# microsoft/MoGe

Hardware: AMD Instinct MI355X
Metric: images/sec (MoGeModel.infer, moge-2-vitl 518x518 fp16) (higher is better)
Workload: dtype f16; 1 GPU; moge-2-vitl infer(): batch 32/GPU x 3x518x518 torch.rand, num_tokens 3600, fp16 weights, synthetic checkpoint (seed 0), inputs resident in HBM, outputs left on device; global_batch=32, parallelism=dp1 (independent shards, one-time RCCL weight broadcast)

## Files before the change

include/moge_hip.h:

```cpp
#ifndef MOGE_HIP_H
#define MOGE_HIP_H

#include <stddef.h>
#include <stdint.h>

#ifdef __cplusplus
extern "C" {
#endif

#define MOGE_ABI_VERSION 5
#define MOGE_MAX_TAPS 8
#define MOGE_LEVELS 5

typedef enum moge_status {
    MOGE_OK = 0,
    MOGE_ERR_INVALID = -1,
    MOGE_ERR_HIP = -2,
    MOGE_ERR_NOT_LOADED = -3,
    MOGE_ERR_MISSING_KEY = -4,
    MOGE_ERR_NONFINITE = -5
} moge_status;

typedef enum moge_precision {
    MOGE_FP32 = 0,
// ... 124 lines not shown
int moge_cast_f16(const float* src, void* dst_f16, int64_t n, void* stream);

int moge_sync(moge_handle* h, void* stream);

int moge_profile_enable(moge_handle* h, int on);
int moge_profile_read(moge_handle* h, moge_profile* out, int reset);

int moge_debug_tap(moge_handle* h, const char* name, float* dst, int64_t dst_capacity, int64_t* numel, void* stream);

void moge_tune_set(const char* key, int value);

int moge_test_gemm(int precision, const float* A, const float* W, const float* bias, float* C, int M, int N, int K,
                   int act, void* stream);
enum { MOGE_TG_STORE = 0, MOGE_TG_RESID = 1, MOGE_TG_QKV = 2, MOGE_TG_CONVT = 3, MOGE_TG_PATCH = 4 };
typedef struct moge_test_gemm_args {
    int32_t precision, kind, act;
    int32_t M, N, K;
    const float* A; const float* W; const float* bias;
    float* out;
    const float* ln_mr; const float* ln_c;
    const float* wu; const float* wv; float u0, u1, v0, v1;
    int32_t pixW, pixH, Cout;
    float* xres; const float* gamma; float* x16_out; float* ln_part_out;
    float* q_out; float* k_out; float* v_out; int32_t nh, Ntok; float qscale;
    const float* pos; const float* cls; int32_t Np;
    int32_t v_transposed;
    int32_t uv_in;
} moge_test_gemm_args;
int moge_test_gemm_ex(const moge_test_gemm_args* args, void* stream);
int moge_test_layernorm(int precision, const float* x, const float* w, const float* b, float* y, int rows, int D, void* stream);
int moge_test_attention(int precision, const float* q, const float* k, const float* v, float* o, int B, int nh, int N, void* stream);
int moge_test_conv3x3(int precision, const float* x, const float* w, const float* bias, float* y, int B, int H, int W,
                      int Cin, int Cout, int relu_in, void* stream);
typedef struct moge_test_conv_args {
    int32_t precision, B, H, W, Cin, Cout;
    int32_t relu_in, act, up2;
    const float* x; const float* w; const float* bias;
    const float* add;
    const float* side; const float* side_w;
    const float* wu; const float* wv; float u0, u1, v0, v1;
    const float* w2; const float* bias2;
    float* y;
    const float* dot_w; int32_t dot_rows;
} moge_test_conv_args;
int moge_test_conv_ex(const moge_test_conv_args* args, void* stream);
typedef struct moge_test_ct3_args {
    int32_t precision, B, H, W, Cin, Cout, no_border;
    const float* x; const float* wt; const float* bt; const float* w3; const float* b3;
    const float* side; const float* side_w;
    const float* wu; const float* wv; float u0, u1, v0, v1;
    float* y;
} moge_test_ct3_args;
int moge_test_ct3(const moge_test_ct3_args* args, void* stream);
int moge_test_convt2x2(int precision, const float* x, const float* w, const float* bias, float* y, int B, int H, int W,
                       int Cin, int Cout, void* stream);
int moge_test_preprocess(const float* image, float* out, int B, int H, int W, int rows, int cols, void* stream);
int moge_test_preprocess_ex(int in_fp16, int out_fp16, const float* image, float* out, int32_t* zero_i32, int B, int H, int W, int rows, int cols, int ldk,
                            int nchw_out, int round16, int aa, int zero_n, void* stream);
int moge_test_resize_bicubic_aa(const float* image, float* out, int B, int H, int W, int OH, int OW, void* stream);
int moge_test_resize_bicubic_aa_ex(int in_fp16, const float* image, float* out, int B, int H, int W, int OH, int OW, int round16, void* stream);
int moge_test_groupnorm_relu(int precision, const float* x, const float* gamma, const float* beta, float* y, int B, int H, int W, int C, int groups, void* stream);
int moge_test_norm_act(int precision, const float* x, const float* gamma, const float* beta, float* y, int B, int H, int W, int C, int groups, int act, int in_place, void* stream);
int moge_test_posembed(const float* pos, float* out, int D, int rows, int cols, void* stream);
int moge_test_posembed_ex(const float* pos, float* out, int D, int rows, int cols, int size_mode, void* stream);
int moge_test_recover(const float* points, const uint8_t* mask, const float* focal_in, int B, int H, int W,
                      float* focal, float* shift, int32_t* status, void* stream);
typedef struct moge_test_head_args {
    int32_t precision, kind, remap, ksize;
    int32_t B, Hd, Wd, C, ld, choff, H, W;
    int32_t n4_below;
    const float* x; const float* w; const float* bias;
    const float* n4; const float* w2;
    float* out;
} moge_test_head_args;
int moge_test_head_final(const moge_test_head_args* args, void* stream);
int moge_test_head_final_dot(int kind, int remap, const float* y, const float* z, int zld, int zoff, const float* bias, float* out, int B, int Hd, int Wd,
                             int H, int W, void* stream);
int moge_test_mlp_layer(const float* in, const float* W, const float* bias, float* out, int B, int K, int N, int act, void* stream);
int moge_test_layernorm_ex(int precision, int stream16, const float* x, const float* w, const float* b, float* y, float* cls_out, int rows, int D, int ldo,
                           int coloff, int tap_mode, int Ntok, void* stream);
int moge_test_ln_raw(const float* x, float* x16_out, float* mr, int rows, int D, void* stream);
int moge_test_ln_finalize(const float* part, float* mr, int rows, int NP, int D, void* stream);
int moge_test_fold_ln(const float* W, const float* g, const float* beta, const float* b, float* Wf_out, float* c, float* bf, int N, int K, void* stream);
int moge_test_resize_bilinear_uv(int precision, const float* x, float* out, int B, int hs, int ws, int C, int OH, int OW, int Cp, float u0, float u1,
                                 float v0, float v1, void* stream);
int moge_test_u8_ingest(int precision, const uint8_t* in, float* out, int B, int H, int W, void* stream);

int moge_align_l1(const float* x, const float* y, const float* w, int rows, int n, float eps, float* a, float* loss, int32_t* index, void* stream);
int moge_align_l1_anchored(const float* src, const float* tgt, const float* weight, int n, int d, int comp_mask, const int32_t* row_batch,
                           const int32_t* row_anchor, int rows, float eps, float* scale, float* loss, int32_t* index, void* stream);
int moge_align_trunc_workspace(int n, int rows, int64_t* bytes);
int moge_align_trunc(const float* x, const float* y, const float* w, int rows, int n, float trunc, float eps, void* workspace, float* a, float* loss,
                     int32_t* index, void* stream);
int moge_align_trunc_anchored(const float* src, const float* tgt, const float* weight, int n, int d, int comp_mask, const int32_t* row_batch,
                              const int32_t* row_anchor, int rows, float trunc, float eps, void* workspace, float* scale, float* loss, int32_t* index,
                              void* stream);
int moge_align_select(const float* loss, const int32_t* row_batch, int rows, int batch, float* min_loss, int32_t* min_row, void* stream);
int moge_align_lstsq(const float* x, const float* y, const float* w, int rows, int n, float* a, float* b, void* stream);

#define MOGE_METRICS_PARTIALS 256
#define MOGE_METRICS_MAX_SEGMENTS 512
int moge_metrics_lr_sample(const uint8_t* mask, int H, int W, int out_h, int out_w, uint8_t* lr_mask, int32_t* lr_index, void* stream);
int moge_metrics_error(const float* pred, const float* gt, const uint8_t* mask, int n, int dim, const float* params, int K, double* partials,
                       double* out, void* stream);
int moge_metrics_masked_max(const float* x, const uint8_t* mask, int n, float* partials, float* out, void* stream);
int moge_metrics_boundary(const float* pred, const float* gt, const uint8_t* mask, int H, int W, int64_t* counts, void* stream);
// ... 46 lines not shown
```

moge_amd/_lib.py:

```python
from __future__ import annotations

import ctypes as C
import os

import torch

HERE = os.path.dirname(os.path.abspath(__file__))
LIB_PATH = os.path.join(HERE, "lib", "libmoge_hip.so")
EXPERIMENTS_LIB_PATH = os.path.join(HERE, "lib", "experiments", "libmoge_hip.so")

MOGE_MAX_TAPS = 8
MOGE_LEVELS = 5
FP32, FP16, FP16_HALF = 0, 1, 2
HEAD_POINTS, HEAD_NORMAL, HEAD_MASK, HEAD_SCALE = 1, 2, 4, 8
FORCE_PROJECTION, APPLY_MASK = 1, 2
REMAP = {"linear": 0, "sinh": 1, "exp": 2, "sinh_exp": 3}
RESAMPLER = {"conv_transpose": 0, "bilinear": 1, "nearest": 2, "pixel_shuffle": 3}
RES_NORM = {"none": 0, "layer_norm": 1, "group_norm": 2, "instance_norm": 3}
ACTIVATION = {"relu": 0, "leaky_relu": 1, "silu": 2, "elu": 3}
ERR_NONFINITE = -5
KC_NAMES = ["gemm", "attn", "conv", "norm", "pre", "post", "recover", "gemm_pp"]
ABI_VERSION = 5
MESH_MAX_MAPS, MESH_BLOCK_PX, MESH_SCAN_SPAN, MESH_NO_FACES = 8, 1024, 256, -1
MESH_F32, MESH_U8, MESH_UV = 0, 1, 2
# ... 62 lines not shown
                ("B", C.c_int32), ("Hd", C.c_int32), ("Wd", C.c_int32), ("C", C.c_int32), ("ld", C.c_int32), ("choff", C.c_int32), ("H", C.c_int32), ("W", C.c_int32),
                ("n4_below", C.c_int32), ("x", C.c_void_p), ("w", C.c_void_p), ("bias", C.c_void_p), ("n4", C.c_void_p), ("w2", C.c_void_p), ("out", C.c_void_p)]


class MeshMap(C.Structure):
    _fields_ = [("data", C.c_void_p), ("out", C.c_void_p), ("channels", C.c_int32), ("dtype", C.c_int32), ("has_scale", C.c_int32),
                ("has_offset", C.c_int32), ("scale", C.c_float * 4), ("offset", C.c_float * 4)]


class MogeError(RuntimeError):
    pass


def _load(path: str = LIB_PATH, mode: int = C.RTLD_GLOBAL) -> C.CDLL:
    if not os.path.exists(path):
        raise ImportError(f"{path} is missing: build it with `python -m moge_amd.build` (hipcc, gfx950). "
                          "moge_amd has no CPU / PyTorch fallback.")
    lib = C.CDLL(path, mode=mode)
    vp, i32, i64, f32p = C.c_void_p, C.c_int, C.c_int64, C.c_void_p
    sig = {
        "moge_abi_version": (C.c_int, []),
        "moge_last_error": (C.c_char_p, []),
        "moge_create": (C.c_int, [C.POINTER(MogeConfig), i32, C.POINTER(vp)]),
        "moge_create_v1": (C.c_int, [C.POINTER(MogeV1Config), i32, C.POINTER(vp)]),
        "moge_v1_forward": (C.c_int, [vp, vp, i32, i32, i32, i32, i32, i32, C.POINTER(Outputs), vp]),
        "moge_v1_infer": (C.c_int, [vp, vp, i32, i32, i32, i32, i32, i32, vp, i32, C.POINTER(Outputs), vp]),
        "moge_destroy": (None, [vp]),
        "moge_load_weights": (C.c_int, [vp, C.POINTER(TensorDesc), i32, vp]),
        "moge_alloc_master": (C.c_int, [vp]),
        "moge_master_blob": (C.c_int, [vp, C.POINTER(vp), C.POINTER(C.c_size_t)]),
        "moge_master_ready": (C.c_int, [vp]),
        "moge_broadcast_weights": (C.c_int, [vp, vp, i32, vp]),
        "moge_set_precision": (C.c_int, [vp, i32, vp]),
        "moge_set_onnx_compatible_mode": (C.c_int, [vp, i32]),
        "moge_workspace_bytes": (C.c_int, [vp, i32, i32, i32, i32, i32, C.POINTER(C.c_size_t)]),
        "moge_forward": (C.c_int, [vp, vp, i32, i32, i32, i32, i32, i32, C.POINTER(Outputs), vp]),
        "moge_infer": (C.c_int, [vp, vp, i32, i32, i32, i32, i32, i32, vp, i32, C.POINTER(Outputs), vp]),
        "moge_postprocess": (C.c_int, [vp, vp, vp, vp, vp, i32, i32, i32, vp, i32, C.POINTER(Outputs), vp]),
        "moge_depth_edge_mask": (C.c_int, [vp, vp, vp, i32, i32, i32, C.c_float, vp, vp]),
        "moge_cast_f16": (C.c_int, [vp, vp, C.c_int64, vp]),
        "moge_sync": (C.c_int, [vp, vp]),
        "moge_profile_enable": (C.c_int, [vp, i32]),
        "moge_profile_read": (C.c_int, [vp, C.POINTER(Profile), i32]),
        "moge_debug_tap": (C.c_int, [vp, C.c_char_p, vp, i64, C.POINTER(i64), vp]),
        "moge_tune_set": (None, [C.c_char_p, i32]),
        "moge_test_gemm": (C.c_int, [i32, f32p, f32p, f32p, f32p, i32, i32, i32, i32, vp]),
        "moge_test_gemm_ex": (C.c_int, [C.POINTER(TestGemmArgs), vp]),
        "moge_test_layernorm": (C.c_int, [i32, f32p, f32p, f32p, f32p, i32, i32, vp]),
        "moge_test_attention": (C.c_int, [i32, f32p, f32p, f32p, f32p, i32, i32, i32, vp]),
        "moge_test_conv3x3": (C.c_int, [i32, f32p, f32p, f32p, f32p, i32, i32, i32, i32, i32, i32, vp]),
        "moge_test_conv_ex": (C.c_int, [C.POINTER(TestConvArgs), vp]),
        "moge_test_convt2x2": (C.c_int, [i32, f32p, f32p, f32p, f32p, i32, i32, i32, i32, i32, vp]),
        "moge_test_ct3": (C.c_int, [C.POINTER(TestCt3Args), vp]),
        "moge_test_preprocess": (C.c_int, [f32p, f32p, i32, i32, i32, i32, i32, vp]),
        "moge_test_preprocess_ex": (C.c_int, [i32, i32, f32p, f32p, vp, i32, i32, i32, i32, i32, i32, i32, i32, i32, i32, vp]),
        "moge_test_resize_bicubic_aa": (C.c_int, [f32p, f32p, i32, i32, i32, i32, i32, vp]),
        "moge_test_resize_bicubic_aa_ex": (C.c_int, [i32, f32p, f32p, i32, i32, i32, i32, i32, i32, vp]),
        "moge_test_groupnorm_relu": (C.c_int, [i32, f32p, f32p, f32p, f32p, i32, i32, i32, i32, i32, vp]),
        "moge_test_norm_act": (C.c_int, [i32, f32p, f32p, f32p, f32p, i32, i32, i32, i32, i32, i32, i32, vp]),
        "moge_test_posembed": (C.c_int, [f32p, f32p, i32, i32, i32, vp]),
        "moge_test_posembed_ex": (C.c_int, [f32p, f32p, i32, i32, i32, i32, vp]),
        "moge_test_recover": (C.c_int, [f32p, vp, f32p, i32, i32, i32, f32p, f32p, vp, vp]),
        "moge_test_head_final": (C.c_int, [C.POINTER(TestHeadArgs), vp]),
        "moge_test_head_final_dot": (C.c_int, [i32, i32, f32p, f32p, i32, i32, f32p, f32p, i32, i32, i32, i32, i32, vp]),
        "moge_test_mlp_layer": (C.c_int, [f32p, f32p, f32p, f32p, i32, i32, i32, i32, vp]),
        "moge_test_layernorm_ex": (C.c_int, [i32, i32, f32p, f32p, f32p, f32p, f32p, i32, i32, i32, i32, i32, i32, vp]),
        "moge_test_ln_raw": (C.c_int, [f32p, f32p, f32p, i32, i32, vp]),
        "moge_test_ln_finalize": (C.c_int, [f32p, f32p, i32, i32, i32, vp]),
        "moge_test_fold_ln": (C.c_int, [f32p, f32p, f32p, f32p, f32p, f32p, f32p, i32, i32, vp]),
        "moge_test_resize_bilinear_uv": (C.c_int, [i32, f32p, f32p, i32, i32, i32, i32, i32, i32, i32, C.c_float, C.c_float, C.c_float, C.c_float, vp]),
        "moge_test_u8_ingest": (C.c_int, [i32, vp, f32p, i32, i32, i32, vp]),
        "moge_align_l1": (C.c_int, [f32p, f32p, f32p, i32, i32, C.c_float, f32p, f32p, vp, vp]),
        "moge_align_l1_anchored": (C.c_int, [f32p, f32p, f32p, i32, i32, i32, vp, vp, i32, C.c_float, f32p, f32p, vp, vp]),
        "moge_align_trunc_workspace": (C.c_int, [i32, i32, C.POINTER(i64)]),
        "moge_align_trunc": (C.c_int, [f32p, f32p, f32p, i32, i32, C.c_float, C.c_float, vp, f32p, f32p, vp, vp]),
        "moge_align_trunc_anchored": (C.c_int, [f32p, f32p, f32p, i32, i32, i32, vp, vp, i32, C.c_float, C.c_float, vp, f32p, f32p, vp, vp]),
        "moge_align_select": (C.c_int, [f32p, vp, i32, i32, f32p, vp, vp]),
        "moge_align_lstsq": (C.c_int, [f32p, f32p, f32p, i32, i32, f32p, f32p, vp]),
        "moge_metrics_lr_sample": (C.c_int, [vp, i32, i32, i32, i32, vp, vp, vp]),
        "moge_metrics_error": (C.c_int, [vp, vp, vp, i32, i32, vp, i32, vp, vp, vp]),
        "moge_metrics_masked_max": (C.c_int, [vp, vp, i32, vp, vp, vp]),
        "moge_metrics_boundary": (C.c_int, [vp, vp, vp, i32, i32, vp, vp]),
        "moge_metrics_segment_stats": (C.c_int, [vp, vp, vp, i32, i32, vp, vp, i32, i32, vp, i32, vp, vp, vp, vp]),
        "moge_metrics_segment_pack": (C.c_int, [vp, i32, vp, vp, i32, i32, vp, i32, vp, i32, i32, vp, vp, vp, vp, vp, vp, vp]),
        "moge_metrics_segment_error": (C.c_int, [vp, vp, vp, vp, i32, vp, i32, vp, vp, i32, vp, vp, vp, vp, vp, vp]),
        "moge_eval_lanczos_workspace": (C.c_int, [i32, i32, i32, i32, vp, vp]),
        "moge_eval_lanczos": (C.c_int, [vp, i32, i32, i32, i32, vp, vp, vp, vp]),
        "moge_eval_masked_nearest": (C.c_int, [vp, vp, i32, i32, i32, i32, C.c_float, C.c_float, C.c_float, C.c_float, vp, vp, vp, vp]),
        "moge_eval_resize_nearest": (C.c_int, [vp, i32, i32, i32, i32, i32, vp, vp]),
        "moge_eval_remap": (C.c_int, [vp, vp, vp, vp, i32, i32, i32, i32, i32, f32p, vp, vp, vp, vp, vp, vp, vp]),
        "moge_eval_quantile_cut": (C.c_int, [vp, vp, i32, C.c_float, C.c_float, C.c_float, i32, vp, vp, vp]),
        "moge_eval_unproject": (C.c_int, [vp, vp, i32, i32, f32p, vp, vp, vp]),
        "moge_refine_depth_workspace": (C.c_int, [i32, i32, i32, C.POINTER(i64)]),
        "moge_refine_depth": (C.c_int, [f32p, f32p, f32p, vp, i32, i32, i32, i32, i32, C.c_float, C.c_float, vp, f32p, vp]),
        "moge_image_mesh_workspace": (C.c_int, [i32, i32, i32, C.POINTER(i64)]),
        "moge_image_mesh_count": (C.c_int, [vp, i32, i32, i32, i32, vp, vp, vp, vp]),
        "moge_image_mesh_fill": (C.c_int, [i32, i32, i32, vp, C.POINTER(MeshMap), i32, i32, vp, vp, vp]),
    }
    for name, (res, args) in sig.items():
        fn = getattr(lib, name)
        fn.restype = res
        fn.argtypes = args
    if lib.moge_abi_version() != ABI_VERSION:
        raise ImportError("libmoge_hip.so ABI version mismatch")
    return lib


lib = _load()
_experiments_lib = None


def experiments_lib() -> C.CDLL:
    global _experiments_lib
    if _experiments_lib is None:
        _experiments_lib = _load(EXPERIMENTS_LIB_PATH, C.RTLD_LOCAL)
    return _experiments_lib
EXPORTS = ["moge_abi_version", "moge_last_error", "moge_create", "moge_create_v1", "moge_v1_forward", "moge_v1_infer", "moge_destroy", "moge_load_weights", "moge_alloc_master",
           "moge_master_blob", "moge_master_ready", "moge_broadcast_weights", "moge_set_precision", "moge_set_onnx_compatible_mode", "moge_workspace_bytes", "moge_forward", "moge_infer",
           "moge_postprocess", "moge_depth_edge_mask", "moge_cast_f16", "moge_sync", "moge_profile_enable", "moge_profile_read", "moge_debug_tap", "moge_tune_set", "moge_test_gemm",
           "moge_test_gemm_ex", "moge_test_layernorm", "moge_test_attention", "moge_test_conv3x3", "moge_test_conv_ex", "moge_test_convt2x2", "moge_test_ct3", "moge_test_preprocess",
           "moge_test_resize_bicubic_aa", "moge_test_groupnorm_relu", "moge_test_norm_act", "moge_test_posembed", "moge_test_recover",
           "moge_test_head_final", "moge_test_head_final_dot", "moge_test_mlp_layer", "moge_test_layernorm_ex", "moge_test_ln_raw", "moge_test_ln_finalize",
           "moge_test_fold_ln", "moge_test_resize_bilinear_uv", "moge_test_u8_ingest",
           "moge_test_preprocess_ex", "moge_test_posembed_ex", "moge_test_resize_bicubic_aa_ex",
           "moge_align_l1", "moge_align_l1_anchored", "moge_align_trunc_workspace", "moge_align_trunc", "moge_align_trunc_anchored",
           "moge_align_select", "moge_align_lstsq",
           "moge_metrics_lr_sample", "moge_metrics_error", "moge_metrics_masked_max", "moge_metrics_boundary", "moge_metrics_segment_stats",
           "moge_metrics_segment_pack", "moge_metrics_segment_error",
           "moge_eval_lanczos_workspace", "moge_eval_lanczos", "moge_eval_masked_nearest", "moge_eval_resize_nearest", "moge_eval_remap",
           "moge_eval_quantile_cut", "moge_eval_unproject",
           "moge_refine_depth_workspace", "moge_refine_depth",
           "moge_image_mesh_workspace", "moge_image_mesh_count", "moge_image_mesh_fill"]


def check(code: int) -> None:
    if code == 0:
        return
    msg = (lib.moge_last_error() or b"").decode(errors="replace")
    if code == ERR_NONFINITE:
        raise ValueError(msg or "Residuals are not finite in the initial point.")
    raise MogeError(f"libmoge_hip error {code}: {msg}")


def tune(key: str, value: int) -> None:
    lib.moge_tune_set(key.encode(), int(value))


def stream_ptr(device=None) -> int:
    return int(torch.cuda.current_stream(device).cuda_stream)


class DevView:

    def __init__(self, ptr: int, nbytes: int):
        self.__cuda_array_interface__ = {"shape": (nbytes,), "typestr": "|u1", "data": (ptr, False), "version": 2, "strides": None}
```

moge_amd/csrc/conv_pp.hip:

```cpp
#include "common.h"

#define CP_GPTR(p) ((const __attribute__((address_space(1))) void*)(p))
__device__ __forceinline__ unsigned cp_opaque(unsigned v) { asm volatile("" : "+v"(v)); return v; }
#define CP_LPTR(p) ((__attribute__((address_space(3))) void*)(p))

namespace {

template <int TW> struct Halo {
    static constexpr int W = TW + 2;
    static constexpr int PX = 18 * W;
    static constexpr int PIECES = (PX + 7) / 8;
    static constexpr int BYTES = PIECES * 1024;
    static constexpr int HPW = (PIECES + 7) / 8;
};

__device__ __forceinline__ u32x4 relu8(u32x4 v) {
#pragma unroll
    for (int i = 0; i < 4; i++) {
        unsigned t = v[i];
        asm("v_pk_max_f16 %0, %0, 0" : "+v"(t));
        v[i] = t;
    }
    return v;
}

template <int N> __device__ __forceinline__ void wait_vm_lgkm() { asm volatile("s_waitcnt vmcnt(%0) lgkmcnt(0)" ::"n"(N) : "memory"); }

template <int BN, int TW, int NH, int EPI>
__global__ __launch_bounds__(512, (BN == 64 && TW == 16 && NH == 1) ? 4 : 2) void conv_pp_kernel(const GemmArgs g) {
    constexpr bool CONVT = (EPI & 2) != 0, HAS_UV = (EPI & 1) != 0, RELU_IN = (EPI & 4) != 0;
    constexpr bool M16 = (EPI & 8) != 0;
    static_assert(!M16 || TW == 16, "16x16x32 path: 16-pixel-wide tiles");
    constexpr bool SIDE_REG = (EPI & 16) != 0;
    constexpr bool DOT = (EPI & 32) != 0;
    static_assert(!DOT || (CONVT && M16 && BN == 128), "fused output conv: the 64 -> 4 x 32 pixel-shuffle resampler");
    constexpr bool CT3 = (EPI & 64) != 0;
    static_assert(!CT3 || (CONVT && M16 && !DOT && !RELU_IN && !SIDE_REG && NH == 2), "fused ConvTranspose2d + 3x3: pixel-shuffle store, 16x16x32 form, two halo buffers");
    constexpr int NTAP = CT3 ? 4 : 9;
    static_assert(!SIDE_REG || (M16 && BN == 64 && NH == 1), "register side input: single-image 64-channel form");
    constexpr int WN = BN / 64, WM = 8 / WN, TM = TW * 16 / 32 / WM, TN = 2;
    constexpr int HALO_W = Halo<TW>::W, HALO_PX = Halo<TW>::PX, HALO_PIECES = Halo<TW>::PIECES, HALO_BYTES = Halo<TW>::BYTES, HPW = Halo<TW>::HPW;
    constexpr int LOG_TW = TW == 16 ? 4 : 5;
    constexpr bool PERSIST = !(BN == 64 && NH == 1);
    constexpr int NWP = BN / 64;
    constexpr int WSLOT = BN * 128;
    constexpr int LDS_W = NH * HALO_BYTES;
    constexpr int WROWS = TM * 32;
    extern __shared__ __attribute__((aligned(16))) char smem[];

    const int tid = threadIdx.x, lane = tid & 63;
    const int wave = __builtin_amdgcn_readfirstlane(tid >> 6);
    const int grp = wave >> 2;
    const int hi = lane >> 5, l31 = lane & 31;
    const int wm = wave / WN, wn = wave % WN;

    const int H = g.H, W = g.W, C = g.C;
    const int tx_n = (W + TW - 1) / TW, ty_n = (H + 15) >> 4;
    const int nbn = g.N / BN;
    int li, cnt, start, wgs_x;
    {
        const int nwg = gridDim.x;
        const int ntiles = PERSIST ? (g.M / (H * W)) * ty_n * tx_n * nbn : nwg;
        const int nx = nwg < 8 ? nwg : 8, xcd = blockIdx.x % nx;
        const int q = ntiles / nx, r = ntiles % nx;
        cnt = q + (xcd < r ? 1 : 0);
        start = xcd * q + min(xcd, r);
        wgs_x = (nwg - xcd + nx - 1) / nx;
        li = blockIdx.x / nx;
    }
    if (li >= cnt) return;
    int b, y0, x0, n0;
    const int nchunks = NH == 1 ? 1 : (C >> 6);
    const int C2 = CT3 ? g.Cout : C;
    const int nside = SIDE_REG ? 1 : ((NH > 1 && g.a2) ? (C2 >> 6) : 0);
    const int nkt1 = nchunks * NTAP;
    const int nkt = nkt1 + nside;

    const int prow = lane >> 3, pch = lane & 7;
    const char* in_b;
    const char* in2_b;
    const char* w_b;
    const char* w2_b;
    unsigned hoff[HPW];
    unsigned hoff2[CT3 ? HPW : 1];
    int sb, sy0, sx0, sn0;
    auto setup = [&](int idx) {
        int prow_t = prow, pch_t = pch;
        if constexpr (PERSIST) asm volatile("" : "+v"(prow_t), "+v"(pch_t));
        const int wgt = start + idx;
        const int bn_ = wgt % nbn;
        int t = wgt / nbn;
        const int tx = t % tx_n; t /= tx_n;
        const int ty = t % ty_n;
        sb = t / ty_n; sy0 = ty * 16; sx0 = tx * TW; sn0 = bn_ * BN;
        in_b = reinterpret_cast<const char*>(g.a) + (size_t)sb * H * W * C * 2;
        in2_b = reinterpret_cast<const char*>(g.a2) + (size_t)sb * H * W * C2 * (CT3 ? 8 : 2);
        w_b = reinterpret_cast<const char*>(g.w) + (size_t)sn0 * g.ldw * 2;
        w2_b = reinterpret_cast<const char*>(g.w2) + (CT3 ? (size_t)0 : (size_t)sn0 * C * 2);
        const int spy = CT3 ? (sn0 / BN) >> 1 : 0, spx = CT3 ? (sn0 / BN) & 1 : 0;
#pragma unroll
        for (int i = 0; i < HPW; i++) {
            int piece = wave + 8 * i;
            piece = piece < HALO_PIECES ? piece : HALO_PIECES - 1;
            int hp = piece * 8 + prow_t;
            const int sw = ((EPI & 8) ? (hp % HALO_W) : ((hp % HALO_W) >> 1)) & 7;
            hp = hp < HALO_PX ? hp : HALO_PX - 1;
            const int hy = hp / HALO_W, hx = hp - hy * HALO_W;
            int yy = sy0 - 1 + hy, xx = sx0 - 1 + hx;
            yy = yy < 0 ? 0 : (yy > H - 1 ? H - 1 : yy);
            xx = xx < 0 ? 0 : (xx > W - 1 ? W - 1 : xx);
            hoff[i] = (unsigned)(((yy * W + xx) * C) * 2 + ((pch_t ^ sw) << 4));
            if constexpr (CT3) hoff2[i] = (unsigned)((((2 * yy + spy) * (2 * W) + 2 * xx + spx) * C2) * 2 + ((pch_t ^ sw) << 4));
        }
    };
    int wrow[NWP];
    unsigned wsw[NWP];
#pragma unroll
    for (int i = 0; i < NWP; i++) {
        wrow[i] = (wave + 8 * i) * 8 + prow;
        wsw[i] = (unsigned)((pch ^ ((wrow[i] >> 1) & 7)) << 4);
    }
    auto issue_halo = [&](int c) {
        char* dst = smem + (c & (NH - 1)) * HALO_BYTES;
        const char* src = uniform_ptr(c < nchunks ? in_b + (size_t)c * 128 : in2_b + (size_t)(c - nchunks) * 128);
        const bool side2 = CT3 && c >= nchunks;
#pragma unroll
        for (int i = 0; i < HPW; i++) {
            int piece = wave + 8 * i;
            piece = piece < HALO_PIECES ? piece : HALO_PIECES - 1;
            unsigned off = hoff[i];
            if constexpr (CT3) off = side2 ? hoff2[i] : off;
            __builtin_amdgcn_global_load_lds(CP_GPTR(src + cp_opaque(off)), CP_LPTR(dst + piece * 1024), 16, 0, 0);
        }
    };
    auto issue_w = [&](int kt) {
        char* dst = smem + LDS_W + (kt & 3) * WSLOT;
        const bool side = kt >= nkt1;
        const int c = CT3 ? kt >> 2 : kt / 9, tap = CT3 ? kt & 3 : kt - c * 9;
        const char* src = uniform_ptr(side ? w2_b + (size_t)(kt - nkt1) * 128 : w_b + ((size_t)tap * C + c * 64) * 2);
        const int rowb = side ? C2 * 2 : g.ldw * 2;
#pragma unroll
        for (int i = 0; i < NWP; i++) {
            const unsigned off = (unsigned)(wrow[i] * rowb) + wsw[i];
            __builtin_amdgcn_global_load_lds(CP_GPTR(src + cp_opaque(off)), CP_LPTR(dst + (wave + 8 * i) * 1024), 16, 0, 0);
        }
    };

    int hp0[TM], hx0[TM];
#pragma unroll
    for (int i = 0; i < TM; i++) {
        const int mp = wm * WROWS + i * 32 + l31;
        hx0[i] = (mp & (TW - 1)) + 1;
        hp0[i] = ((mp >> LOG_TW) + 1) * HALO_W + hx0[i];
    }
    const int sxw = (l31 >> 1) & 7;
    const int w_off = (wn * 64 + l31) * 128 + ((hi ^ sxw) << 4);
    const int l15 = lane & 15, g4 = lane >> 4;
    const int w_off16 = (wn * 64 + l15) * 128 + ((g4 ^ ((l15 >> 1) & 7)) << 4);

    f32x16 acc[TM][TN];
    f32x4 acc16[2 * TM][4];
    const int ntot = nchunks + nside;
    int kt = 0, halo_age = 2;
    int l15t = l15;
    int abase[3][2];
    int tpy = 0;
    auto set_abase = [&]() {
        const bool ph2 = CT3 && BN == 2 * g.Cout;
        const int tpx = CT3 ? (ph2 ? wn : (n0 / BN) & 1) : 0;
        if constexpr (CT3) tpy = ph2 ? (n0 / BN) & 1 : (n0 / BN) >> 1;
#pragma unroll
        for (int d = 0; d < 3; d++) {
            const int hx = l15t + (CT3 ? (d == 2 ? 1 : tpx + d) : d);
            const int a = wm * (2 * TM * HALO_W * 128) + hx * 128 + ((g4 ^ (hx & 7)) << 4);
            abase[d][0] = a; abase[d][1] = a ^ 64;
        }
    };
    u32x4 sidef[SIDE_REG ? 2 * TM : 1][2];
    auto kstep = [&](const char* halo, int dy, int dx, bool first_of_image, int image, bool relu, bool from_regs = false) {
        const char* wsl = smem + LDS_W + (kt & 3) * WSLOT;
        u32x4 af[TM][4], wf[TN][4];
        if constexpr (M16) {
            if (from_regs) {
                if constexpr (SIDE_REG) {
#pragma unroll
                    for (int i = 0; i < 2 * TM; i++)
#pragma unroll
                        for (int ks = 0; ks < 2; ks++) af[i >> 1][(i & 1) * 2 + ks] = sidef[i][ks];
                }
            } else {
#pragma unroll
            for (int i = 0; i < 2 * TM; i++) {
#pragma unroll
                for (int ks = 0; ks < 2; ks++)
                    af[i >> 1][(i & 1) * 2 + ks] = *reinterpret_cast<const u32x4*>(halo + abase[dx + 1][ks] + (i + 1 + dy) * (HALO_W * 128));
            }
            }
#pragma unroll
            for (int j = 0; j < 4; j++)
#pragma unroll
                for (int ks = 0; ks < 2; ks++) wf[j >> 1][(j & 1) * 2 + ks] = *reinterpret_cast<const u32x4*>(wsl + (w_off16 ^ (ks * 64)) + j * 2048);
        } else {
#pragma unroll
        for (int i = 0; i < TM; i++) {
            const int hp = hp0[i] + dy * HALO_W + dx;
            const int a0 = hp * 128 + ((hi ^ (((hx0[i] + dx) >> 1) & 7)) << 4);
#pragma unroll
            for (int ks = 0; ks < 4; ks++) af[i][ks] = *reinterpret_cast<const u32x4*>(halo + (a0 ^ (ks * 32)));
        }
#pragma unroll
        for (int j = 0; j < TN; j++)
#pragma unroll
            for (int ks = 0; ks < 4; ks++) wf[j][ks] = *reinterpret_cast<const u32x4*>(wsl + (w_off ^ (ks * 32)) + j * 4096);
        }
        const bool halo_now = NH > 1 && first_of_image && image + 1 < ntot;
        if (halo_now) { issue_halo(image + 1); halo_age = 0; }
        const int ahead = nkt - 2 - kt;
        if (ahead >= 2) issue_w(kt + 3);
        if (halo_now && image >= nchunks) {
            if (ahead >= 2) wait_vm_lgkm<NWP>();
            else wait_vm_lgkm<0>();
        } else if (NH > 1 && halo_age <= 1) {
            if (ahead >= 2) wait_vm_lgkm<2 * NWP + HPW>();
            else if (ahead == 1) wait_vm_lgkm<NWP + HPW>();
            else wait_vm_lgkm<HPW>();
        } else {
            if (ahead >= 2) wait_vm_lgkm<2 * NWP>();
            else if (ahead == 1) wait_vm_lgkm<NWP>();
            else wait_vm_lgkm<0>();
        }
        halo_age++;
        if constexpr (RELU_IN) {
            if (relu) {
#pragma unroll
                for (int i = 0; i < TM; i++)
#pragma unroll
                    for (int ks = 0; ks < 4; ks++) af[i][ks] = relu8(af[i][ks]);
            }
        }
        __builtin_amdgcn_s_barrier();
        asm volatile("" ::: "memory");
        __builtin_amdgcn_sched_barrier(0);
        __builtin_amdgcn_s_setprio(1);
        if constexpr (M16) {
#pragma unroll
            for (int ks = 0; ks < 2; ks++)
#pragma unroll
                for (int i = 0; i < 2 * TM; i++)
#pragma unroll
                    for (int j = 0; j < 4; j++) mma16<f16>(acc16[i][j], wf[j >> 1][(j & 1) * 2 + ks], af[i >> 1][(i & 1) * 2 + ks]);
        } else {
#pragma unroll
        for (int ks = 0; ks < 4; ks++)
#pragma unroll
            for (int i = 0; i < TM; i++)
#pragma unroll
                for (int j = 0; j < TN; j++) mma_step<f16>(acc[i][j], wf[j][ks], af[i][ks]);
        }
        __builtin_amdgcn_s_setprio(0);
        __builtin_amdgcn_sched_barrier(0);
        asm volatile("" ::: "memory");
        if (!(grp == 1 && kt == nkt - 1)) __builtin_amdgcn_s_barrier();
        asm volatile("" ::: "memory");
        __builtin_amdgcn_sched_barrier(0);
        kt++;
    };
    setup(li);
    if constexpr (SIDE_REG) {
#pragma unroll
        for (int i = 0; i < 2 * TM; i++) {
            int y = sy0 + wm * 2 * TM + i, x = sx0 + l15;
            y = y < H ? y : H - 1; x = x < W ? x : W - 1;
            const char* sp = in2_b + ((size_t)y * W + x) * C * 2 + g4 * 16;
#pragma unroll
            for (int ks = 0; ks < 2; ks++) sidef[i][ks] = *reinterpret_cast<const u32x4*>(sp + ks * 64);
        }
    }
    issue_halo(0);
    bool first = true;
    for (;;) {
    b = sb; y0 = sy0; x0 = sx0; n0 = sn0;
    if constexpr (PERSIST) { asm volatile("" : "+v"(l15t)); if constexpr (M16) set_abase(); }
    else if constexpr (M16) set_abase();
#pragma unroll
    for (int i = 0; i < TM; i++)
#pragma unroll
        for (int j = 0; j < TN; j++)
#pragma unroll
            for (int r = 0; r < 16; r++) acc[i][j][r] = 0.f;
#pragma unroll
    for (int i = 0; i < 2 * TM; i++)
#pragma unroll
        for (int j = 0; j < 4; j++) acc16[i][j] = f32x4{0.f, 0.f, 0.f, 0.f};

    if (!first) {
        asm volatile("s_waitcnt lgkmcnt(0)" ::: "memory");
        __builtin_amdgcn_s_barrier();
        asm volatile("" ::: "memory");
    }
    first = false;
    kt = 0; halo_age = 2;
    issue_w(0);
    issue_w(1);
    issue_w(2);
    wait_vm_lgkm<2 * NWP>();
    __builtin_amdgcn_s_barrier();
    if (grp == 1) __builtin_amdgcn_s_barrier();
    asm volatile("" ::: "memory");
    __builtin_amdgcn_sched_barrier(0);

    for (int c = 0; c < nchunks; c++) {
        const char* halo = smem + (c & (NH - 1)) * HALO_BYTES;
        if constexpr (CT3) {
            const char* hp = halo + tpy * (HALO_W * 128);
#pragma unroll
            for (int tap = 0; tap < 4; tap++) kstep(hp, (tap >> 1) - 1, (tap & 1) - 1, tap == 0, c, true);
        } else {
#pragma unroll
        for (int tap = 0; tap < 9; tap++) kstep(halo, tap / 3 - 1, tap % 3 - 1, tap == 0, c, true);
        }
    }
    if constexpr (SIDE_REG) kstep(smem, 0, 0, false, nchunks, false, true);
    else
    for (int c2 = 0; c2 < nside; c2++) kstep(smem + ((nchunks + c2) & (NH - 1)) * HALO_BYTES, 0, CT3 ? 1 : 0, true, nchunks + c2, false);

    char* R = smem + (PERSIST ? LDS_W : 0) + wave * (WROWS * 128);
    int rr = lane >> 3, cc = lane & 7;
    if constexpr (PERSIST) asm volatile("" : "+v"(rr), "+v"(cc));
    const int nw = n0 + wn * 64;
    const float lo = g.act == ACT_RELU ? 0.f : -3.0e38f;
    const bool has_bias = g.bias != nullptr;
    f16* const outp = reinterpret_cast<f16*>(g.out);
    const f16* const addp = reinterpret_cast<const f16*>(g.add);
    f16x8 addv[WROWS / 8];
    auto load_skip_rows = [&]() {
        if constexpr (!CONVT) {
            if (addp) {
    #pragma unroll
                for (int it = 0; it < WROWS / 8; it++) {
                    const int mp = wm * WROWS + it * 8 + rr;
                    int y = y0 + (mp >> LOG_TW), x = x0 + (mp & (TW - 1));
                    y = y < H ? y : H - 1; x = x < W ? x : W - 1;
                    addv[it] = *reinterpret_cast<const f16x8*>(addp + (((size_t)b * H + y) * W + x) * g.ldadd + nw + cc * 8);
                }
            }
        }
    };
    if constexpr (PERSIST) load_skip_rows();
    u32x4 dota[DOT ? 3 : 1], dotb[DOT ? 2 * TM : 1][2];
    if constexpr (DOT) {
#pragma unroll
        for (int gq = 0; gq < 3; gq++)
            dota[gq] = *reinterpret_cast<const u32x4*>(reinterpret_cast<const char*>(g.dot_tab) + (gq < g.dot_nd ? gq : 0) * 1024 + lane * 16);
    }
    if constexpr (M16) {
        float u0[2 * TM], u1[2 * TM], v0[2 * TM], v1[2 * TM];
        if constexpr (HAS_UV) {
#pragma unroll
            for (int i = 0; i < 2 * TM; i++) {
                int y = y0 + wm * 2 * TM + i, x = x0 + l15;
                y = y < H ? y : H - 1; x = x < W ? x : W - 1;
                if constexpr (CONVT) {
                    u0[i] = linspace_at(g.uv.u0, g.uv.u1, g.uv.ustep, 2 * W, 2 * x);
                    u1[i] = linspace_at(g.uv.u0, g.uv.u1, g.uv.ustep, 2 * W, 2 * x + 1);
                    v0[i] = linspace_at(g.uv.v0, g.uv.v1, g.uv.vstep, 2 * H, 2 * y);
                    v1[i] = linspace_at(g.uv.v0, g.uv.v1, g.uv.vstep, 2 * H, 2 * y + 1);
                } else {
                    u0[i] = u1[i] = linspace_at(g.uv.u0, g.uv.u1, g.uv.ustep, W, x);
                    v0[i] = v1[i] = linspace_at(g.uv.v0, g.uv.v1, g.uv.vstep, H, y);
                }
            }
        }
        f32x4 bvs[4];
#pragma unroll
        for (int jj = 0; jj < 4; jj++) bvs[jj] = *reinterpret_cast<const f32x4*>(g.bias + nw + jj * 16 + 4 * g4);
// ... 59 lines not shown
#pragma unroll
        for (int i = 0; i < TM; i++) {
            const int mp = wm * WROWS + i * 32 + l31;
            int y = y0 + (mp >> LOG_TW), x = x0 + (mp & (TW - 1));
            y = y < H ? y : H - 1; x = x < W ? x : W - 1;
            if constexpr (CONVT) {
                u0[i] = linspace_at(g.uv.u0, g.uv.u1, g.uv.ustep, 2 * W, 2 * x);
                u1[i] = linspace_at(g.uv.u0, g.uv.u1, g.uv.ustep, 2 * W, 2 * x + 1);
                v0[i] = linspace_at(g.uv.v0, g.uv.v1, g.uv.vstep, 2 * H, 2 * y);
                v1[i] = linspace_at(g.uv.v0, g.uv.v1, g.uv.vstep, 2 * H, 2 * y + 1);
            } else {
                u0[i] = u1[i] = linspace_at(g.uv.u0, g.uv.u1, g.uv.ustep, W, x);
                v0[i] = v1[i] = linspace_at(g.uv.v0, g.uv.v1, g.uv.vstep, H, y);
            }
        }
    }
#pragma unroll
    for (int j = 0; j < TN; j++)
#pragma unroll
        for (int q = 0; q < 4; q++) {
            const int n = nw + j * 32 + 8 * q + 4 * hi;
            f32x4 bv = {0.f, 0.f, 0.f, 0.f};
            if (has_bias) bv = *reinterpret_cast<const f32x4*>(g.bias + n);
            f32x4 wu = {0.f, 0.f, 0.f, 0.f}, wv = wu;
            int pdy = 0, pdx = 0;
            if constexpr (HAS_UV) {
                int nco = n;
                if constexpr (CONVT) { const int qd = n / g.Cout; nco = n - qd * g.Cout; pdy = qd >> 1; pdx = qd & 1; }
                wu = *reinterpret_cast<const f32x4*>(g.uv.wu + nco);
                wv = *reinterpret_cast<const f32x4*>(g.uv.wv + nco);
            }
#pragma unroll
            for (int i = 0; i < TM; i++) {
                const int row = i * 32 + l31;
                float v[4];
#pragma unroll
                for (int e = 0; e < 4; e++) v[e] = acc[i][j][4 * q + e] + bv[e];
                if constexpr (HAS_UV) {
                    const float uu = pdx ? u1[i] : u0[i];
                    const float vq = pdy ? v1[i] : v0[i];
#pragma unroll
                    for (int e = 0; e < 4; e++) v[e] += wu[e] * uu + wv[e] * vq;
                }
#pragma unroll
                for (int e = 0; e < 4; e++) v[e] = fmaxf(v[e], lo);
                const f16x4 hv = {(f16)v[0], (f16)v[1], (f16)v[2], (f16)v[3]};
                *reinterpret_cast<f16x4*>(R + row * 128 + ((((j * 4 + q) ^ (row & 7)) << 4) | (hi << 3))) = hv;
            }
        }
    }
    if constexpr (!PERSIST) load_skip_rows();
    bool more = false;
    if constexpr (PERSIST) {
        li += wgs_x;
        more = li < cnt;
        if (more) setup(li);
        __builtin_amdgcn_s_waitcnt(0x0F70);
        if (more) issue_halo(0);
        asm volatile("" ::: "memory");
    }
    if constexpr (!DOT)
#pragma unroll
    for (int it = 0; it < WROWS / 8; it++) {
        const int row = it * 8 + rr;
        const int mp = wm * WROWS + row;
        const int y = y0 + (mp >> LOG_TW), x = x0 + (mp & (TW - 1));
        u32x4 v = *reinterpret_cast<const u32x4*>(R + row * 128 + ((cc ^ (row & 7)) << 4));
        if (y < H && x < W) {
            if constexpr (CONVT) {
                const int n = nw + cc * 8;
                const int qd = n / g.Cout, co = n - qd * g.Cout, pdy = qd >> 1, pdx = qd & 1;
                const size_t idx = ((((size_t)b * 2 * H + 2 * y + pdy) * (2 * W)) + 2 * x + pdx) * g.Cout + co;
                *reinterpret_cast<u32x4*>(outp + idx) = v;
            } else {
                const size_t idx = (((size_t)b * H + y) * W + x) * g.ldc + nw + cc * 8;
                if (addp) {
                    f16x8 h = __builtin_bit_cast(f16x8, v);
                    h += addv[it];
                    v = __builtin_bit_cast(u32x4, h);
                }
                *reinterpret_cast<u32x4*>(outp + idx) = v;
            }
        }
    }
    if (!more) break;
    }
}

template <int BN, int TW, int NH, int EPI>
int launch_conv_cfg(const GemmArgs& g, hipStream_t st) {
    constexpr int smem = NH * Halo<TW>::BYTES + 4 * BN * 128;
    constexpr auto kern = conv_pp_kernel<BN, TW, NH, EPI>;
    if (int rc = set_dyn_lds<kern>(smem)) return rc;
    const long B = (long)g.M / ((long)g.H * g.W);
    const long tiles = B * ((g.H + 15) / 16) * ((g.W + TW - 1) / TW) * (g.N / BN);
    const int ncu = pp_device_cus();
    long slots = (BN == 64 && NH == 1) ? tiles : (long)ncu;
    const long cap = moge_tune_get("CONV_GRID", 0);
    if (cap > 0 && !(BN == 64 && NH == 1)) slots = cap;
    const long grid = tiles < slots ? tiles : slots;
    hipLaunchKernelGGL(kern, dim3((unsigned)grid), dim3(512), smem, st, g);
    return (int)hipGetLastError();
}

}

bool conv_pp_eligible(const GemmArgs& g) {
    if (g.ct3) {
        if ((g.C & 63) || g.K != 4 * g.C || g.ldw != 4 * g.C || !g.bias || g.epi != EPI_CONVT || g.N != 4 * g.Cout) return false;
        if (g.Cout != 128 && g.Cout != 64) return false;
        if (g.add || g.act != ACT_NONE || g.relu_in || g.dot_tab || (g.a2 && !g.w2)) return false;
        if (g.a2 && g.Cout == 64) return false;
        if (g.H < 1 || g.W < 1 || (long)g.M % ((long)g.H * g.W) != 0) return false;
        if ((long)g.H * g.W * g.C * 2 >= (1L << 31) || (long)g.H * g.W * g.Cout * 8 >= (1L << 31)) return false;
        return true;
    }
    if ((g.C & 63) || g.K != 9 * g.C || g.ldw != 9 * g.C || !g.bias) return false;
    if (g.N != 64 && (g.N & 127)) return false;
    if (g.H < 1 || g.W < 1 || (long)g.M % ((long)g.H * g.W) != 0) return false;
    if ((long)g.H * g.W * g.C * 2 >= (1L << 31)) return false;
    if (g.a2 && (!g.w2 || g.epi != EPI_STORE)) return false;
    if (g.relu_in && (g.uv.wu || g.epi != EPI_STORE)) return false;
    if (g.epi == EPI_STORE)
        return (g.ldc & 7) == 0 && (!g.add || ((g.ldadd & 7) == 0 && g.act == ACT_NONE)) && (!g.uv.wu || g.bias) && g.act != ACT_GELU;
    if (g.dot_tab && !(g.epi == EPI_CONVT && g.Cout == 32 && g.N == 128 && g.C == 64 && g.dot_out && g.dot_nd >= 1 && g.dot_nd <= 3 && !g.a2)) return false;
    if (g.epi == EPI_CONVT) return !g.add && g.act == ACT_NONE && (g.Cout == 32 || (g.Cout & 63) == 0) && g.N == 4 * g.Cout;
    return false;
}

template <int BN, int TW, int NH>
static int launch_conv_epi(const GemmArgs& g, hipStream_t st) {
    const int e = (g.uv.wu ? 1 : 0) | (g.epi == EPI_CONVT ? 2 : 0) | (g.relu_in ? 4 : 0);
    if constexpr (BN == 64 && TW == 16 && NH == 1) {
        if (g.a2) return e == 0 ? launch_conv_cfg<BN, TW, NH, 8 | 16>(g, st) : -1;
    }
    if constexpr (BN == 128 && TW == 16 && NH == 1) {
        if (g.dot_tab) {
            if (e == 2) return launch_conv_cfg<BN, TW, NH, 8 | 2 | 32>(g, st);
            if (e == 3) return launch_conv_cfg<BN, TW, NH, 8 | 2 | 1 | 32>(g, st);
            return -1;
        }
    }
#ifdef MOGE_EXPERIMENTS
    if (TW == 32 || moge_tune_get("CONV_M16", 1) == 0) {
        switch (e) {
        case 0: return launch_conv_cfg<BN, TW, NH, 0>(g, st);
        case 1: return launch_conv_cfg<BN, TW, NH, 1>(g, st);
        case 2: return launch_conv_cfg<BN, TW, NH, 2>(g, st);
        case 3: return launch_conv_cfg<BN, TW, NH, 3>(g, st);
        case 4: return launch_conv_cfg<BN, TW, NH, 4>(g, st);
        default: return -1;
        }
    }
#endif
    if constexpr (TW == 16) {
        switch (e) {
        case 0: return launch_conv_cfg<BN, TW, NH, 8>(g, st);
        case 1: return launch_conv_cfg<BN, TW, NH, 9>(g, st);
        case 2: return launch_conv_cfg<BN, TW, NH, 10>(g, st);
        case 3: return launch_conv_cfg<BN, TW, NH, 11>(g, st);
        case 4: return launch_conv_cfg<BN, TW, NH, 12>(g, st);
        default: return -1;
        }
    }
    return -1;
// ... 28 lines not shown
        Y = (cls & 2) ? 2 * H - 1 : 0; X = (cls & 1) ? 2 * W - 1 : 0;
        cy0 = cy1 = (cls & 2) ? H - 1 : 0; cx0 = cx1 = (cls & 1) ? W - 1 : 0;
    }
    f32x4 acc[NJ];
#pragma unroll
    for (int j = 0; j < NJ; j++) acc[j] = f32x4{0.f, 0.f, 0.f, 0.f};
    const f16* wbase = dw + ((size_t)cls * Cout + l15) * (2 * Cin) + 8 * g4;
    const int nslot = cls < 8 ? 2 : 1;
    const int nkc = Cin >> 5, nsteps = nslot * nkc;
    for (int stp = wave; stp < nsteps; stp += 4) {
        const int slot = stp >= nkc ? 1 : 0, kc = (stp - slot * nkc) << 5;
        const f16* pp = in + (((size_t)b * H + (slot ? cy1 : cy0)) * W + (slot ? cx1 : cx0)) * Cin + 8 * g4;
        const f16* wp = wbase + slot * Cin;
        const u32x4 pf = *reinterpret_cast<const u32x4*>(pp + kc);
#pragma unroll
        for (int j = 0; j < NJ; j++) {
            const u32x4 wf = *reinterpret_cast<const u32x4*>(wp + (size_t)j * 16 * (2 * Cin) + kc);
            mma16<f16>(acc[j], wf, pf);
        }
    }
    if (wave > 0) {
#pragma unroll
        for (int j = 0; j < NJ; j++) red[wave - 1][j][lane] = acc[j];
    }
    __syncthreads();
    if (wave > 0) return;
#pragma unroll
    for (int w = 0; w < 3; w++)
#pragma unroll
        for (int j = 0; j < NJ; j++) {
            const f32x4 p = red[w][j][lane];
#pragma unroll
            for (int e = 0; e < 4; e++) acc[j][e] += p[e];
        }
    if (!valid) return;
    f16* op = out + (((size_t)b * 2 * H + Y) * (2 * W) + X) * Cout + 4 * g4;
#pragma unroll
    for (int j = 0; j < NJ; j++) {
        f16x4 v = *reinterpret_cast<const f16x4*>(op + j * 16);
        v = f16x4{(f16)((float)v[0] + acc[j][0]), (f16)((float)v[1] + acc[j][1]), (f16)((float)v[2] + acc[j][2]), (f16)((float)v[3] + acc[j][3])};
        *reinterpret_cast<f16x4*>(op + j * 16) = v;
    }
}

int launch_ct3_border(const void* in, const void* dw, void* out, int B, int H, int W, int Cin, int Cout, hipStream_t st) {
    if ((Cin & 31) || (Cout != 128 && Cout != 64) || H < 1 || W < 1) return -1;
    const long mmax = (long)B * ((W > H ? W : H) - 1 > 1 ? (W > H ? W : H) - 1 : 1);
    const dim3 grid((unsigned)((mmax + 15) / 16), 12);
    if (Cout == 128) hipLaunchKernelGGL(ct3_border_kernel<8>, grid, dim3(256), 0, st, (const f16*)in, (const f16*)dw, (f16*)out, B, H, W, Cin);
    else hipLaunchKernelGGL(ct3_border_kernel<4>, grid, dim3(256), 0, st, (const f16*)in, (const f16*)dw, (f16*)out, B, H, W, Cin);
    return (int)hipGetLastError();
}

int launch_conv_pp(const GemmArgs& g, hipStream_t st) {
    if (g.ct3) {
        return g.uv.wu ? launch_conv_cfg<128, 16, 2, 8 | 2 | 64 | 1>(g, st) : launch_conv_cfg<128, 16, 2, 8 | 2 | 64>(g, st);
    }
    const bool side_reg = g.C == 64 && g.N == 64 && g.a2 && !g.uv.wu && !g.relu_in && g.epi == EPI_STORE && moge_tune_get("CONV_SIDE_REG", 1);
    const bool one_image = g.C == 64 && (!g.a2 || side_reg);
    if (g.N == 64) {
#ifdef MOGE_EXPERIMENTS
        if (one_image && g.W >= 32 && moge_tune_get("CONV_TW32", 0)) return launch_conv_epi<64, 32, 1>(g, st);
#endif
        return one_image ? launch_conv_epi<64, 16, 1>(g, st) : launch_conv_epi<64, 16, 2>(g, st);
    }
    return one_image ? launch_conv_epi<128, 16, 1>(g, st) : launch_conv_epi<128, 16, 2>(g, st);
}
```

Measured before the change: 249.0 images/s.

## Pair both output-row phases per CT3 tile and add register side input for 64-channel

For the fused ConvTranspose2d+3x3 kernel with Cin=128, Cout=64, each persistent tile now runs two passes (one per output-row phase) over the same loaded input halo, instead of treating the two N-blocks as separate tiles. This avoids reloading the halo for the second pass. A new SIDE2 variant loads the side (skip) input straight into registers, which lets the Cout=64 case with a side input use the fused path instead of falling back. The change adds pass-state control flow to the persistent loop and more register pressure, and the pairing is switched on by default through a tune flag.

```diff
diff --git a/include/moge_hip.h b/include/moge_hip.h
--- a/include/moge_hip.h
+++ b/include/moge_hip.h
@@ -200,6 +200,7 @@
     float* y;
 } moge_test_ct3_args;
 int moge_test_ct3(const moge_test_ct3_args* args, void* stream);
+int moge_test_ct3_ex(const moge_test_ct3_args* args, int flags, void* stream);
 int moge_test_convt2x2(int precision, const float* x, const float* w, const float* bias, float* y, int B, int H, int W,
                        int Cin, int Cout, void* stream);
 int moge_test_preprocess(const float* image, float* out, int B, int H, int W, int rows, int cols, void* stream);
diff --git a/moge_amd/_lib.py b/moge_amd/_lib.py
--- a/moge_amd/_lib.py
+++ b/moge_amd/_lib.py
@@ -138,6 +138,7 @@
         "moge_test_conv_ex": (C.c_int, [C.POINTER(TestConvArgs), vp]),
         "moge_test_convt2x2": (C.c_int, [i32, f32p, f32p, f32p, f32p, i32, i32, i32, i32, i32, vp]),
         "moge_test_ct3": (C.c_int, [C.POINTER(TestCt3Args), vp]),
+        "moge_test_ct3_ex": (C.c_int, [C.POINTER(TestCt3Args), i32, vp]),
         "moge_test_preprocess": (C.c_int, [f32p, f32p, i32, i32, i32, i32, i32, vp]),
         "moge_test_preprocess_ex": (C.c_int, [i32, i32, f32p, f32p, vp, i32, i32, i32, i32, i32, i32, i32, i32, i32, i32, vp]),
         "moge_test_resize_bicubic_aa": (C.c_int, [f32p, f32p, i32, i32, i32, i32, i32, vp]),
@@ -204,7 +205,7 @@
 EXPORTS = ["moge_abi_version", "moge_last_error", "moge_create", "moge_create_v1", "moge_v1_forward", "moge_v1_infer", "moge_destroy", "moge_load_weights", "moge_alloc_master",
            "moge_master_blob", "moge_master_ready", "moge_broadcast_weights", "moge_set_precision", "moge_set_onnx_compatible_mode", "moge_workspace_bytes", "moge_forward", "moge_infer",
            "moge_postprocess", "moge_depth_edge_mask", "moge_cast_f16", "moge_sync", "moge_profile_enable", "moge_profile_read", "moge_debug_tap", "moge_tune_set", "moge_test_gemm",
-           "moge_test_gemm_ex", "moge_test_layernorm", "moge_test_attention", "moge_test_conv3x3", "moge_test_conv_ex", "moge_test_convt2x2", "moge_test_ct3", "moge_test_preprocess",
+           "moge_test_gemm_ex", "moge_test_layernorm", "moge_test_attention", "moge_test_conv3x3", "moge_test_conv_ex", "moge_test_convt2x2", "moge_test_ct3", "moge_test_ct3_ex", "moge_test_preprocess",
            "moge_test_resize_bicubic_aa", "moge_test_groupnorm_relu", "moge_test_norm_act", "moge_test_posembed", "moge_test_recover",
            "moge_test_head_final", "moge_test_head_final_dot", "moge_test_mlp_layer", "moge_test_layernorm_ex", "moge_test_ln_raw", "moge_test_ln_finalize",
            "moge_test_fold_ln", "moge_test_resize_bilinear_uv", "moge_test_u8_ingest",
diff --git a/moge_amd/csrc/conv_pp.hip b/moge_amd/csrc/conv_pp.hip
--- a/moge_amd/csrc/conv_pp.hip
+++ b/moge_amd/csrc/conv_pp.hip
@@ -36,6 +36,10 @@
     static_assert(!DOT || (CONVT && M16 && BN == 128), "fused output conv: the 64 -> 4 x 32 pixel-shuffle resampler");
     constexpr bool CT3 = (EPI & 64) != 0;
     static_assert(!CT3 || (CONVT && M16 && !DOT && !RELU_IN && !SIDE_REG && NH == 2), "fused ConvTranspose2d + 3x3: pixel-shuffle store, 16x16x32 form, two halo buffers");
+    constexpr bool SIDE2 = (EPI & 128) != 0;
+    static_assert(!SIDE2 || (CT3 && BN == 128), "register side input of the two-phase CT3 form");
+    const bool pair = CT3 && g.ct3 == 2;
+    int pass = 0;
     constexpr int NTAP = CT3 ? 4 : 9;
     static_assert(!SIDE_REG || (M16 && BN == 64 && NH == 1), "register side input: single-image 64-channel form");
     constexpr int WN = BN / 64, WM = 8 / WN, TM = TW * 16 / 32 / WM, TN = 2;
@@ -56,7 +60,7 @@
 
     const int H = g.H, W = g.W, C = g.C;
     const int tx_n = (W + TW - 1) / TW, ty_n = (H + 15) >> 4;
-    const int nbn = g.N / BN;
+    const int nbn = pair ? 1 : g.N / BN;
     int li, cnt, start, wgs_x;
     {
         const int nwg = gridDim.x;
@@ -72,7 +76,7 @@
     int b, y0, x0, n0;
     const int nchunks = NH == 1 ? 1 : (C >> 6);
     const int C2 = CT3 ? g.Cout : C;
-    const int nside = SIDE_REG ? 1 : ((NH > 1 && g.a2) ? (C2 >> 6) : 0);
+    const int nside = (SIDE_REG || SIDE2) ? 1 : ((NH > 1 && g.a2) ? (C2 >> 6) : 0);
     const int nkt1 = nchunks * NTAP;
     const int nkt = nkt1 + nside;
 
@@ -82,7 +86,7 @@
     const char* w_b;
     const char* w2_b;
     unsigned hoff[HPW];
-    unsigned hoff2[CT3 ? HPW : 1];
+    unsigned hoff2[(CT3 && !SIDE2) ? HPW : 1];
     int sb, sy0, sx0, sn0;
     auto setup = [&](int idx) {
         int prow_t = prow, pch_t = pch;
@@ -110,7 +114,7 @@
             yy = yy < 0 ? 0 : (yy > H - 1 ? H - 1 : yy);
             xx = xx < 0 ? 0 : (xx > W - 1 ? W - 1 : xx);
             hoff[i] = (unsigned)(((yy * W + xx) * C) * 2 + ((pch_t ^ sw) << 4));
-            if constexpr (CT3) hoff2[i] = (unsigned)((((2 * yy + spy) * (2 * W) + 2 * xx + spx) * C2) * 2 + ((pch_t ^ sw) << 4));
+            if constexpr (CT3 && !SIDE2) hoff2[i] = (unsigned)((((2 * yy + spy) * (2 * W) + 2 * xx + spx) * C2) * 2 + ((pch_t ^ sw) << 4));
         }
     };
     int wrow[NWP];
@@ -129,7 +133,7 @@
             int piece = wave + 8 * i;
             piece = piece < HALO_PIECES ? piece : HALO_PIECES - 1;
             unsigned off = hoff[i];
-            if constexpr (CT3) off = side2 ? hoff2[i] : off;
+            if constexpr (CT3 && !SIDE2) off = side2 ? hoff2[i] : off;
             __builtin_amdgcn_global_load_lds(CP_GPTR(src + cp_opaque(off)), CP_LPTR(dst + piece * 1024), 16, 0, 0);
         }
     };
@@ -141,7 +145,7 @@
         const int rowb = side ? C2 * 2 : g.ldw * 2;
 #pragma unroll
         for (int i = 0; i < NWP; i++) {
-            const unsigned off = (unsigned)(wrow[i] * rowb) + wsw[i];
+            const unsigned off = (unsigned)(((SIDE2 && side) ? (wrow[i] & 63) : wrow[i]) * rowb) + wsw[i];
             __builtin_amdgcn_global_load_lds(CP_GPTR(src + cp_opaque(off)), CP_LPTR(dst + (wave + 8 * i) * 1024), 16, 0, 0);
         }
     };
@@ -160,7 +164,7 @@
 
     f32x16 acc[TM][TN];
     f32x4 acc16[2 * TM][4];
-    const int ntot = nchunks + nside;
+    const int ntot = SIDE2 ? nchunks : nchunks + nside;
     int kt = 0, halo_age = 2;
     int l15t = l15;
     int abase[3][2];
@@ -176,13 +180,23 @@
             abase[d][0] = a; abase[d][1] = a ^ 64;
         }
     };
-    u32x4 sidef[SIDE_REG ? 2 * TM : 1][2];
+    u32x4 sidef[(SIDE_REG || SIDE2) ? 2 * TM : 1][2];
+    auto load_side2 = [&](int spy) {
+#pragma unroll
+        for (int i = 0; i < 2 * TM; i++) {
+            int y = sy0 + wm * 2 * TM + i, x = sx0 + l15;
+            y = y < H ? y : H - 1; x = x < W ? x : W - 1;
+            const char* sp = in2_b + (((size_t)(2 * y + spy) * (2 * W) + 2 * x + wn) * C2) * 2 + g4 * 16;
+#pragma unroll
+            for (int ks = 0; ks < 2; ks++) sidef[i][ks] = *reinterpret_cast<const u32x4*>(sp + ks * 64);
+        }
+    };
     auto kstep = [&](const char* halo, int dy, int dx, bool first_of_image, int image, bool relu, bool from_regs = false) {
         const char* wsl = smem + LDS_W + (kt & 3) * WSLOT;
         u32x4 af[TM][4], wf[TN][4];
         if constexpr (M16) {
             if (from_regs) {
-                if constexpr (SIDE_REG) {
+                if constexpr (SIDE_REG || SIDE2) {
 #pragma unroll
                     for (int i = 0; i < 2 * TM; i++)
 #pragma unroll
@@ -213,7 +227,7 @@
 #pragma unroll
             for (int ks = 0; ks < 4; ks++) wf[j][ks] = *reinterpret_cast<const u32x4*>(wsl + (w_off ^ (ks * 32)) + j * 4096);
         }
-        const bool halo_now = NH > 1 && first_of_image && image + 1 < ntot;
+        const bool halo_now = NH > 1 && first_of_image && image + 1 < ntot && !(CT3 && pass == 1);
         if (halo_now) { issue_halo(image + 1); halo_age = 0; }
         const int ahead = nkt - 2 - kt;
         if (ahead >= 2) issue_w(kt + 3);
@@ -276,10 +290,14 @@
             for (int ks = 0; ks < 2; ks++) sidef[i][ks] = *reinterpret_cast<const u32x4*>(sp + ks * 64);
         }
     }
+    if constexpr (SIDE2) load_side2((sn0 / BN) & 1);
     issue_halo(0);
     bool first = true;
     for (;;) {
     b = sb; y0 = sy0; x0 = sx0; n0 = sn0;
+    if constexpr (CT3) {
+        if (pair) { n0 = pass * BN; w_b = reinterpret_cast<const char*>(g.w) + (size_t)n0 * g.ldw * 2; }
+    }
     if constexpr (PERSIST) { asm volatile("" : "+v"(l15t)); if constexpr (M16) set_abase(); }
     else if constexpr (M16) set_abase();
 #pragma unroll
@@ -320,7 +338,7 @@
         for (int tap = 0; tap < 9; tap++) kstep(halo, tap / 3 - 1, tap % 3 - 1, tap == 0, c, true);
         }
     }
-    if constexpr (SIDE_REG) kstep(smem, 0, 0, false, nchunks, false, true);
+    if constexpr (SIDE_REG || SIDE2) kstep(smem, 0, 0, false, nchunks, false, true);
     else
     for (int c2 = 0; c2 < nside; c2++) kstep(smem + ((nchunks + c2) & (NH - 1)) * HALO_BYTES, 0, CT3 ? 1 : 0, true, nchunks + c2, false);
 
@@ -486,12 +504,17 @@
     if constexpr (!PERSIST) load_skip_rows();
     bool more = false;
     if constexpr (PERSIST) {
-        li += wgs_x;
-        more = li < cnt;
-        if (more) setup(li);
+        const bool adv = !(CT3 && pair && pass == 0);
+        if (adv) {
+            li += wgs_x;
+            more = li < cnt;
+            if (more) setup(li);
+        }
         __builtin_amdgcn_s_waitcnt(0x0F70);
-        if (more) issue_halo(0);
+        if (adv && more) issue_halo(0);
         asm volatile("" ::: "memory");
+        if constexpr (SIDE2) { if (!adv) load_side2(1); else if (more) load_side2((sn0 / BN) & 1); asm volatile("" ::: "memory"); }
+        if constexpr (CT3) { if (!adv) more = true; pass = adv ? 0 : 1; }
     }
     if constexpr (!DOT)
 #pragma unroll
@@ -527,7 +550,7 @@
     constexpr auto kern = conv_pp_kernel<BN, TW, NH, EPI>;
     if (int rc = set_dyn_lds<kern>(smem)) return rc;
     const long B = (long)g.M / ((long)g.H * g.W);
-    const long tiles = B * ((g.H + 15) / 16) * ((g.W + TW - 1) / TW) * (g.N / BN);
+    const long tiles = B * ((g.H + 15) / 16) * ((g.W + TW - 1) / TW) * (g.ct3 == 2 ? 1 : g.N / BN);
     const int ncu = pp_device_cus();
     long slots = (BN == 64 && NH == 1) ? tiles : (long)ncu;
     const long cap = moge_tune_get("CONV_GRID", 0);
@@ -544,7 +567,6 @@
         if ((g.C & 63) || g.K != 4 * g.C || g.ldw != 4 * g.C || !g.bias || g.epi != EPI_CONVT || g.N != 4 * g.Cout) return false;
         if (g.Cout != 128 && g.Cout != 64) return false;
         if (g.add || g.act != ACT_NONE || g.relu_in || g.dot_tab || (g.a2 && !g.w2)) return false;
-        if (g.a2 && g.Cout == 64) return false;
         if (g.H < 1 || g.W < 1 || (long)g.M % ((long)g.H * g.W) != 0) return false;
         if ((long)g.H * g.W * g.C * 2 >= (1L << 31) || (long)g.H * g.W * g.Cout * 8 >= (1L << 31)) return false;
         return true;
@@ -679,8 +701,11 @@
     return (int)hipGetLastError();
 }
 
-int launch_conv_pp(const GemmArgs& g, hipStream_t st) {
+int launch_conv_pp(const GemmArgs& g_in, hipStream_t st) {
+    GemmArgs g = g_in;
     if (g.ct3) {
+        g.ct3 = (g.Cout == 64 && g.C == 128 && moge_tune_get("CT3_PY_PAIR", 1)) ? 2 : 1;
+        if (g.a2 && g.Cout == 64) return g.uv.wu ? launch_conv_cfg<128, 16, 2, 8 | 2 | 64 | 128 | 1>(g, st) : launch_conv_cfg<128, 16, 2, 8 | 2 | 64 | 128>(g, st);
         return g.uv.wu ? launch_conv_cfg<128, 16, 2, 8 | 2 | 64 | 1>(g, st) : launch_conv_cfg<128, 16, 2, 8 | 2 | 64>(g, st);
     }
     const bool side_reg = g.C == 64 && g.N == 64 && g.a2 && !g.uv.wu && !g.relu_in && g.epi == EPI_STORE && moge_tune_get("CONV_SIDE_REG", 1);
```

After: 250.6 images/s, median of 6. Within noise of the previous version (+0.7%).
